# FunAudioLLM/CosyVoice

Measured on NVIDIA H100. Metric: audio-sec/s, CosyVoice2-0.5B zero-shot batch-32, NFE=10, higher is better.
Workload: dtype bf16

## Files before the change

cosyvoice_b200/csrc/api.cu:

```cuda
#include "common.cuh"
#include <string.h>
#include <algorithm>

void hift_build(cvk_ctx* ctx);
void hift_f0(cvk_ctx* ctx, const float* mel, const int* lens, int B, float* f0_out, cudaStream_t st);
void hift_source(cvk_ctx* ctx, const float* f0, const int* lens, int B, const float* noise, float* source_out, cudaStream_t st);
void hift_decode(cvk_ctx* ctx, const float* mel, const int* lens, int B, const float* source, float* wav, cudaStream_t st);
void hift_inference(cvk_ctx* ctx, const float* mel, const int* lens, int B, const float* noise, const float* cache_source,
                    const int* cache_lens, float* wav, float* source_out, cudaStream_t st);
void flow_build(cvk_ctx* ctx, const int* cfg, int ncfg);
void flow_encoder(cvk_ctx* ctx, const int32_t* tokens, const int* lens, int B, int streaming, int context_len, float* h, cudaStream_t st);
void flow_estimator(cvk_ctx* ctx, const float* x, const float* mu, const float* t, const float* spks, const float* cond, const int* lens,
                    int B, int streaming, float* out, cudaStream_t st);
void flow_cfm_solve(cvk_ctx* ctx, const float* mu, const float* spks, const float* cond, const int* lens, int B, const float* z,
                    int n_timesteps, float cfg_rate, int streaming, float* out, cudaStream_t st);
void flow_inference(cvk_ctx* ctx, const int32_t* tokens, const int* token_lens, const float* prompt_feat, const int* prompt_feat_lens,
                    const float* embedding, int B, int n_timesteps, int streaming, int finalize, float* mel, cudaStream_t st);
void flow_set_noise(cvk_ctx* ctx, const float* noise_tm, int T, int on_device);
void llm_build(cvk_ctx* ctx, const int* cfg, int ncfg);
cvk_lm_session* llm_session_create(cvk_ctx* ctx, int max_batch, int max_context);
void llm_session_destroy(cvk_ctx* ctx, cvk_lm_session* s);
void hift3_build(cvk_ctx* ctx);
void hift3_set_noise(cvk_ctx* ctx, const float* rand_ini, const float* sine_noise, long long n, int on_device);
void hift3_inference(cvk_ctx* ctx, const float* mel, const int* lens, int B, int finalize, float* wav, float* f0_out, float* source_out,
// ... 36 lines not shown
  if (!ctx) return CVK_ERR_INVALID; \
  try {                          \
    cudaSetDevice(ctx->device);
#define CVK_API_END                                  \
    return CVK_OK;                                   \
  } catch (const CvkError& e) {                      \
    ctx->last_error = e.what();                      \
    return e.code;                                   \
  } catch (const std::exception& e) {                \
    ctx->last_error = std::string("internal: ") + e.what(); \
    return CVK_ERR_INVALID;                          \
  }

extern "C" {

const char* cvk_version(void) { return "libcvk 0.1 (sm_90a)"; }

int cvk_create(int device, int precision, size_t workspace_bytes, cvk_ctx** out) {
  if (!out) return CVK_ERR_INVALID;
  *out = nullptr;
  int n = 0;
  if (cudaGetDeviceCount(&n) != cudaSuccess || n <= device || device < 0) return CVK_ERR_CUDA;
  if (precision != CVK_PREC_FP32 && precision != CVK_PREC_BF16) return CVK_ERR_INVALID;
  if (cudaSetDevice(device) != cudaSuccess) return CVK_ERR_CUDA;
  cudaDeviceProp prop;
  if (cudaGetDeviceProperties(&prop, device) != cudaSuccess) return CVK_ERR_CUDA;
  if (prop.major != 9) return CVK_ERR_CUDA;
  cvk_ctx* ctx = new cvk_ctx();
  ctx->device = device;
  ctx->precision = precision;
  ctx->act_dtype = precision == CVK_PREC_BF16 ? DT_BF16 : DT_F32;
  ctx->num_sms = prop.multiProcessorCount;
  if (workspace_bytes == 0) workspace_bytes = (size_t)4 << 30;
  void* p = nullptr;
  if (cudaMalloc(&p, workspace_bytes) != cudaSuccess) {
    delete ctx;
    return CVK_ERR_OOM;
  }
  ctx->arena.base = (char*)p;
  ctx->arena.cap = workspace_bytes;
  *out = ctx;
  return CVK_OK;
}

void cvk_destroy(cvk_ctx* ctx) {
  if (!ctx) return;
  cudaSetDevice(ctx->device);
  cudaDeviceSynchronize();
  for (auto& kv : ctx->raw) cudaFree(kv.second.p);
  for (void* p : ctx->owned) cudaFree(p);
  cudaFree(ctx->arena.base);
  delete ctx;
}

const char* cvk_last_error(cvk_ctx* ctx) { return ctx ? ctx->last_error.c_str() : "null context"; }
thread_local int cvk_in_capture = 0;
int64_t cvk_launch_count(cvk_ctx* ctx) { return ctx ? ctx->launches.load() : 0; }
int cvk_stream_create(cvk_ctx* ctx, void** out) {
  CVK_API_BEGIN
  CVK_REQUIRE(out != nullptr, "cvk_stream_create: bad arguments");
  cudaStream_t s = nullptr;
  CVK_CHECK_CUDA(cudaStreamCreateWithFlags(&s, cudaStreamNonBlocking));
  *out = (void*)s;
  CVK_API_END
}
void cvk_stream_destroy(cvk_ctx* ctx, void* stream) {
  if (!ctx || !stream) return;
  cudaSetDevice(ctx->device);
  cudaStreamDestroy((cudaStream_t)stream);
}
double cvk_last_op_ms(cvk_ctx* ctx) { return ctx ? ctx->op_ms : 0.0; }
int cvk_debug_read(cvk_ctx* ctx, long long* out, int n) {
  if (!ctx || !ctx->tl || !out || n != 4096) return CVK_ERR_INVALID;
  cudaSetDevice(ctx->device);
  if (cudaMemcpy(out, ctx->tl, 4096 * sizeof(long long), cudaMemcpyDeviceToHost) != cudaSuccess) return CVK_ERR_CUDA;
  return CVK_OK;
}

int cvk_set_option(cvk_ctx* ctx, const char* key, int value) {
  CVK_API_BEGIN
  std::string k(key ? key : "");
  if (k == "use_tc") ctx->use_tc = value;
  else if (k == "flow_fused_ff") ctx->flow_fused_ff = value;
  else if (k == "tc_epi") ctx->tc_epi = value;
  else if (k == "tc_persist") ctx->tc_persist = value;
  else if (k == "op_out_bf16") ctx->op_out_bf16 = value;
  else if (k == "op_iters") ctx->op_iters = value;
  else if (k == "use_graph") ctx->use_graph = value;
  else if (k == "use_tc_attn") ctx->use_tc_attn = value;
  else if (k == "use_skinny") ctx->use_skinny = value;
  else if (k == "lm_fused") ctx->lm_fused = value;
  else if (k == "pdl") ctx->pdl = value;
  else if (k == "lm_mega") ctx->lm_mega = value;
  else if (k == "enc_tc_attn") ctx->enc_tc_attn = value;
  else if (k == "hift_f16") ctx->hift_f16 = value;
  else if (k == "mega_coop") ctx->mega_coop = value;
  else if (k == "chain_timeline") {
    if (value && !ctx->tl) {
      ctx->tl = ctx->dmalloc(4096 * sizeof(long long));
      CVK_CHECK_CUDA(cudaMemset(ctx->tl, 0, 4096 * sizeof(long long)));
    }
    if (!value) ctx->tl = nullptr;
  }
  else throw CvkError(CVK_ERR_INVALID, "unknown option: " + k);
  CVK_API_END
}

int cvk_profile(cvk_ctx* ctx, int enable) {
  CVK_API_BEGIN
  CVK_CHECK_CUDA(cudaDeviceSynchronize());
  for (auto& r : ctx->prof) { ctx->event_pool.push_back(r.a); ctx->event_pool.push_back(r.b); }
  ctx->prof.clear();
  ctx->prof_on = enable;
  CVK_API_END
}

int cvk_profile_read(cvk_ctx* ctx, int family, double* ms, double* flops, double* bytes, int64_t* launches) {
  CVK_API_BEGIN
  CVK_REQUIRE(family >= 0 && family < FAM_COUNT && ms && flops && bytes && launches, "cvk_profile_read: bad arguments");
  CVK_CHECK_CUDA(cudaDeviceSynchronize());
  double t = 0, w = 0, by = 0;
  int64_t n = 0;
  for (auto& r : ctx->prof) {
    if (r.family != family) continue;
    float e = 0.f;
    CVK_CHECK_CUDA(cudaEventElapsedTime(&e, r.a, r.b));
    t += e; w += r.work; by += r.bytes; ++n;
  }
  *ms = t; *flops = w; *bytes = by; *launches = n;
  CVK_API_END
}

int cvk_set_tensor(cvk_ctx* ctx, const char* name, const float* data, int on_device, const int64_t* shape, int ndim) {
  CVK_API_BEGIN
  CVK_REQUIRE(name && data && shape && ndim >= 1 && ndim <= 4, "cvk_set_tensor: bad arguments");
  RawTensor t;
  t.shape.assign(shape, shape + ndim);
  size_t bytes = (size_t)t.numel() * sizeof(float);
  CVK_CHECK_CUDA(cudaMalloc((void**)&t.p, bytes));
  cudaError_t e = cudaMemcpy(t.p, data, bytes, on_device ? cudaMemcpyDeviceToDevice : cudaMemcpyHostToDevice);
  if (e != cudaSuccess) {
    cudaFree(t.p);
    throw CvkError(CVK_ERR_CUDA, std::string("cvk_set_tensor copy: ") + cudaGetErrorString(e));
  }
  auto it = ctx->raw.find(name);
  if (it != ctx->raw.end()) {
    cudaFree(it->second.p);
    ctx->raw.erase(it);
  }
  ctx->raw[name] = t;
  CVK_API_END
}

int cvk_finalize(cvk_ctx* ctx, const char* stage, const int* cfg, int ncfg) {
  CVK_API_BEGIN
  std::string s(stage ? stage : "");
  if (s == "hift") hift_build(ctx);
  else if (s == "flow") flow_build(ctx, cfg, ncfg);
  else if (s == "flow3") dit_build(ctx, cfg, ncfg);
  else if (s == "hift3") hift3_build(ctx);
  else if (s == "llm") llm_build(ctx, cfg, ncfg);
  else if (s == "mel") mel_init(ctx);
  else if (s == "prompt") prompt_feat_init(ctx);
  else throw CvkError(CVK_ERR_INVALID, "unknown stage: " + s);
  CVK_CHECK_CUDA(cudaDeviceSynchronize());
  std::string prefix = s + ".";
// ... 632 lines not shown
```

cosyvoice_b200/csrc/cvk_internal.h:

```cpp
#pragma once
#include <cuda_runtime.h>
#include <cuda_bf16.h>
#include <cuda_fp16.h>
#include <cuda.h>
#include <stdint.h>
#include <stdio.h>
#include <string>
#include <vector>
#include <map>
#include <unordered_map>
#include <stdexcept>
#include <atomic>

#include "../../include/cvk.h"

typedef __nv_bfloat16 bf16;

struct CvkError : std::runtime_error {
  int code;
  CvkError(int c, const std::string& m) : std::runtime_error(m), code(c) {}
};

#define CVK_CHECK_CUDA(expr)                                                                       \
  do {                                                                                             \
// ... 73 lines not shown
extern thread_local int cvk_in_capture;

struct Arena {
  char* base = nullptr;
  size_t cap = 0, off = 0, high = 0;
  void* alloc(size_t bytes) {
    size_t a = (off + 255) & ~(size_t)255;
    if (a + bytes > cap) throw CvkError(CVK_ERR_OOM, "workspace arena exhausted: need " + std::to_string(a + bytes) +
                                                          " of " + std::to_string(cap));
    off = a + bytes;
    if (off > high) high = off;
    return base + a;
  }
  void reset() { off = 0; }
};

struct RawTensor {
  float* p = nullptr;
  std::vector<int64_t> shape;
  int64_t numel() const { int64_t n = 1; for (auto s : shape) n *= s; return n; }
};

enum ProfFamily { FAM_GEMM_TC = 0, FAM_GEMM_SIMT = 1, FAM_ATTN = 2, FAM_COUNT = 3 };
struct ProfRec {
  cudaEvent_t a, b;
  int family;
  double work;
  double bytes;
};

struct HiftModel;
struct FlowModel;
struct DitModel;
struct LlmModel;

struct cvk_ctx {
  int device = 0;
  int precision = CVK_PREC_FP32;
  int act_dtype = DT_F32;
  int num_sms = 132;
  std::string last_error;
  std::map<std::string, RawTensor> raw;
  std::vector<void*> owned;
  Arena arena;
  HiftModel* hift = nullptr;
  HiftModel* hift3 = nullptr;
  void* hift3_extra = nullptr;
  FlowModel* flow = nullptr;
  DitModel* dit = nullptr;
  LlmModel* llm = nullptr;
  void* mel_model = nullptr;
  void* prompt_feat_model = nullptr;
  void* encode_tiled = nullptr;
  std::atomic<int64_t> launches{0};
  int op_out_bf16 = 0;
  int op_iters = 0;
  double op_ms = 0.0;
  int tc_epi = 2;
  int tc_persist = 2;
  void* tl = nullptr;
  int tl_seq = 0;
  long long* tl_next() {
    if (!tl) return nullptr;
    long long* p = (long long*)tl + 4 * (tl_seq % 1024);
    ++tl_seq;
    return p;
  }
  int prof_on = 0;
  std::vector<ProfRec> prof;
  std::unordered_map<const void*, void*> tiled;
  std::vector<cudaEvent_t> event_pool;
  int pdl = 1;
  int lm_fused = 1;
  int hift_f16 = 1;
  int build_f16 = 0;
  int enc_tc_attn = 1;
  int lm_mega = 0;
  int mega_coop = 1;
  int use_skinny = 1;
  int use_tc_attn = 1;
  int use_graph = 1;
  int use_tc = 1;
  int flow_fused_ff = 1;

  void* dmalloc(size_t bytes) {
    void* p = nullptr;
    CVK_CHECK_CUDA(cudaMalloc(&p, bytes ? bytes : 16));
    owned.push_back(p);
    return p;
  }
  const RawTensor& get_raw(const std::string& name) const {
    auto it = raw.find(name);
    if (it == raw.end()) throw CvkError(CVK_ERR_MISSING_WEIGHT, "missing weight tensor: " + name);
    return it->second;
  }
  bool has_raw(const std::string& name) const { return raw.find(name) != raw.end(); }
};

template <typename... KArgs, typename... Args>
inline void launch_ex(void (*kern)(KArgs...), dim3 grid, dim3 block, size_t smem, cudaStream_t st, bool pdl, Args&&... args) {
  cudaLaunchConfig_t cfg = {};
  cfg.gridDim = grid;
  cfg.blockDim = block;
  cfg.dynamicSmemBytes = smem;
  cfg.stream = st;
  cudaLaunchAttribute at[1];
  if (pdl) {
    at[0].id = cudaLaunchAttributeProgrammaticStreamSerialization;
    at[0].val.programmaticStreamSerializationAllowed = 1;
    cfg.attrs = at;
    cfg.numAttrs = 1;
  }
  CVK_CHECK_CUDA(cudaLaunchKernelEx(&cfg, kern, KArgs(std::forward<Args>(args))...));
}

Seqs make_seqs(cvk_ctx* ctx, const int* lens, int B, int gap, int scale, int extra_front, cudaStream_t st, bool with_row2seq = true);
Seqs scale_seqs(cvk_ctx* ctx, const Seqs& s, int scale, int extra_front, cudaStream_t st, bool with_row2seq = true);

ConvW make_linear(cvk_ctx* ctx, const std::string& wname, const std::string& bname);
ConvW make_conv(cvk_ctx* ctx, const float* w_oik , const float* bias, int N, int K, int taps,
                int dil, int shift0);
ConvW make_conv_named(cvk_ctx* ctx, const std::string& wname, const std::string& bname, int dil, int shift0);
float* fold_weight_norm(cvk_ctx* ctx, const std::string& prefix, int64_t* numel_out);
void finish_convw(cvk_ctx* ctx, ConvW& w);
float* dev_copy_f32(cvk_ctx* ctx, const float* src_dev, size_t n);

void conv_gemm(cvk_ctx* ctx, cudaStream_t st, const Mat& A, const ConvW& W, const Epilogue& ep);
void conv_gemm_simt(cvk_ctx* ctx, cudaStream_t st, const Mat& A, const ConvW& W, const Epilogue& ep);
void conv_gemm_tc(cvk_ctx* ctx, cudaStream_t st, const Mat& A, const ConvW& W, const Epilogue& ep);
void ffn_fused(cvk_ctx* ctx, cudaStream_t st, const Mat& x, const int* row2seq, const float* ln3_g, const float* ln3_b, const ConvW& w1,
               const ConvW& w2, const float* ln_g, const float* ln_b, const Mat& out);
void flow_ff(cvk_ctx* ctx, cudaStream_t st, const Mat& x, const int* row2seq, const float* ln3_g, const float* ln3_b, const ConvW& ff1,
             const ConvW& ff2, const float* ln_g, const float* ln_b, const Mat& out, const Mat& xn, const Mat& hid);
size_t skinny_scratch_floats(int rows, int maxN);
const bf16* skinny_tiled_weights(cvk_ctx* ctx, const ConvW& W);
void skinny_set_carveout();
int conv_gemm_skinny_ex(cvk_ctx* ctx, cudaStream_t st, const Mat& A, const ConvW& W, const Epilogue& ep, float* scratch, size_t scratch_floats,
                        int mode);
void conv_gemm_skinny(cvk_ctx* ctx, cudaStream_t st, const Mat& A, const ConvW& W, const Epilogue& ep, float* scratch, size_t scratch_floats);

void zero_mat(cvk_ctx* ctx, cudaStream_t st, const Mat& m);
void layernorm(cvk_ctx* ctx, cudaStream_t st, const Mat& x, const float* gamma, const float* beta, float eps, int act,
               float post_scale, const int* row2seq, const Mat& out, const float* rowvec = nullptr, int rowvec_ld = 0);
void unpack_rows_skip(cvk_ctx* ctx, cudaStream_t st, const Mat& in, const Seqs& s, const int* skip_host, float* dense, int C);
Seqs shrink_seqs(cvk_ctx* ctx, const Seqs& s, int drop_tail, cudaStream_t st);
Seqs subseqs(cvk_ctx* ctx, const Seqs& s, const int* skip_host, cudaStream_t st);
void rmsnorm(cvk_ctx* ctx, cudaStream_t st, const Mat& x, const float* gamma, float eps, const Mat& out);
void act_copy(cvk_ctx* ctx, cudaStream_t st, const Mat& x, int act, float param, const float* alpha, const int* row2seq,
              const Mat& out);
void act_copy_scaled(cvk_ctx* ctx, cudaStream_t st, const Mat& x, float pre_scale, int act, float param, const float* alpha,
                     const int* row2seq, const Mat& out);
void pack_rows(cvk_ctx* ctx, cudaStream_t st, const float* dense, int C, const Seqs& s, const Mat& out);
void unpack_rows(cvk_ctx* ctx, cudaStream_t st, const Mat& in, const Seqs& s, int skip, float* dense, int C);
void bcast_rows(cvk_ctx* ctx, cudaStream_t st, const float* vec, int C, int vec_ld, const Seqs& s, const Mat& out);
void convert_mat(cvk_ctx* ctx, cudaStream_t st, const Mat& in, const Mat& out);

struct KvGeom {
  const int* d_kstart = nullptr;
  const int* d_klen = nullptr;
  const int* d_qoff = nullptr;
};
void whisper_log_mel(cvk_ctx* ctx, const float* wav, const int* lens, int B, float* out, cudaStream_t st);
void kaldi_fbank80(cvk_ctx* ctx, const float* wav, const int* lens, int B, int subtract_mean, float* out, cudaStream_t st);
struct cvk_flow_stream;
cvk_flow_stream* flow_stream_create(cvk_ctx* ctx, int kind, int slots, int max_frames, int n_timesteps);
void flow_stream_destroy(cvk_flow_stream* fs);
// ... 44 lines not shown
```

cosyvoice_b200/csrc/gemm_tc.cu:

```cuda
#include "common.cuh"
#include "wgmma.cuh"

namespace {

constexpr int TC_BM = 128;
constexpr int TC_BK = 64;
constexpr int TC_THREADS = 384;

__device__ __forceinline__ uint32_t smem_u32(const void* p) { return (uint32_t)__cvta_generic_to_shared(p); }

__device__ __forceinline__ void mbar_init(uint32_t bar, uint32_t count) {
  asm volatile("mbarrier.init.shared::cta.b64 [%0], %1;" ::"r"(bar), "r"(count));
}
__device__ __forceinline__ void mbar_expect_tx(uint32_t bar, uint32_t bytes) {
  asm volatile("mbarrier.arrive.expect_tx.shared::cta.b64 _, [%0], %1;" ::"r"(bar), "r"(bytes) : "memory");
}
__device__ __forceinline__ void mbar_wait(uint32_t bar, uint32_t parity) {
  uint32_t ok = 0;
  asm volatile(
      "{\n\t.reg .pred p;\n\t"
      "mbarrier.try_wait.parity.shared::cta.b64 p, [%1], %2;\n\t"
      "selp.u32 %0, 1, 0, p;\n\t}"
      : "=r"(ok)
      : "r"(bar), "r"(parity)
// ... 342 lines not shown
      wg_fence();
      if (ep.ab_f16) {
#pragma unroll
        for (int k = 0; k < TC_BK / 16; ++k) wgmma_ss<BN, 1>(acc, da + (uint64_t)(2 * k), db + (uint64_t)(2 * k), 1);
      } else {
#pragma unroll
        for (int k = 0; k < TC_BK / 16; ++k) wgmma_ss<BN, 0>(acc, da + (uint64_t)(2 * k), db + (uint64_t)(2 * k), 1);
      }
      wg_commit();
      wg_wait<1>();
      __syncwarp();
      if (i > 0 && lane == 0) mbar_arrive(smem_u32(&bar_empty[(it - 1) % NSTG]));
    }
    wg_wait<0>();
    wg_touch<BN / 2>(acc);
    __syncwarp();
    if (iters > 0 && lane == 0) mbar_arrive(smem_u32(&bar_empty[(it - 1) % NSTG]));
    asm volatile("bar.sync 1, 256;" ::: "memory");

    const uint32_t stg1 = stg_base;
    const uint32_t stg2 = stg_base + (uint32_t)TC_BM * BN * (ep.out_dtype == DT_F32 ? 4u : 2u);
#pragma unroll
    for (int cb = 0; cb < BN; cb += 32) {
      float a16[16], v[16], w2[16];
      wg_frag_rows16(acc + cb / 2, lane, a16);
      const int c = cb + cq;
      if (n0 + c < N) {
        if (epi_mode == 2) {
          if (n0 + c + 16 <= N) epi_math16p(ep, r, rin, seq, valid, s_bias, c, n0 + c, a16, v, w2);
          else epi_math16(ep, r, rin, n0 + c, N, a16, v, w2);
          stage_store16(stg1, ep.out_dtype, row, c, v);
          if (ep.out2) stage_store16(stg2, ep.out2_dtype, row, c, w2);
        } else if (rin) {
          epi_store16(ep, r, n0 + c, N, a16);
        }
      }
    }
    if (epi_mode == 2) {
      asm volatile("fence.proxy.async.shared::cta;" ::: "memory");
      asm volatile("bar.sync 1, 256;" ::: "memory");
      if (ct == 0) {
        const int w1 = ep.out_dtype == DT_F32 ? 32 : 64;
        for (int sb = 0; sb * w1 < BN && n0 + sb * w1 < N; ++sb) tma_store_2d(&tmap_o, stg1 + sb * 16384u, n0 + sb * w1, r0);
        if (ep.out2) {
          const int w2c = ep.out2_dtype == DT_F32 ? 32 : 64;
          for (int sb = 0; sb * w2c < BN && n0 + sb * w2c < N; ++sb) tma_store_2d(&tmap_o2, stg2 + sb * 16384u, n0 + sb * w2c, r0);
        }
        asm volatile("cp.async.bulk.commit_group;" ::: "memory");
      }
    }
  }
  if (ct == 0 && epi_mode == 2) asm volatile("cp.async.bulk.wait_group 0;" ::: "memory");
}

typedef CUresult (*EncodeTiledFn)(CUtensorMap*, CUtensorMapDataType, cuuint32_t, void*, const cuuint64_t*, const cuuint64_t*,
                                  const cuuint32_t*, const cuuint32_t*, CUtensorMapInterleave, CUtensorMapSwizzle,
                                  CUtensorMapL2promotion, CUtensorMapFloatOOBfill);

EncodeTiledFn get_encode(cvk_ctx* ctx) {
  if (!ctx->encode_tiled) {
    void* fn = nullptr;
    cudaDriverEntryPointQueryResult qres;
    CVK_CHECK_CUDA(cudaGetDriverEntryPoint("cuTensorMapEncodeTiled", &fn, cudaEnableDefault, &qres));
    CVK_REQUIRE(fn != nullptr && qres == cudaDriverEntryPointSuccess, "cuTensorMapEncodeTiled not available");
    ctx->encode_tiled = fn;
  }
  return (EncodeTiledFn)ctx->encode_tiled;
}

template <int BN, int NSTG>
void launch_wg(cvk_ctx* ctx, cudaStream_t st, const CUtensorMap& ta, const CUtensorMap& tw, const CUtensorMap& to, const CUtensorMap& to2,
               const ConvW& W, int rowsOut, const EpiDev& e, int epi_mode) {
  constexpr size_t smem = (size_t)NSTG * (TC_BM * TC_BK * 2 + BN * TC_BK * 2) + TC_STG_BYTES + 1024;
  static bool attr_set = false;
  if (!attr_set) {
    CVK_CHECK_CUDA(cudaFuncSetAttribute(conv_gemm_wg_kernel<BN, NSTG>, cudaFuncAttributeMaxDynamicSharedMemorySize, (int)smem));
    attr_set = true;
  }
  const int ntn = ceil_div(W.N, BN), ntiles = ntn * ceil_div(rowsOut, TC_BM);
  const int grid = (ctx->tc_persist && ntiles > ctx->num_sms) ? ctx->num_sms : ntiles;
  conv_gemm_wg_kernel<BN, NSTG><<<grid, TC_THREADS, smem, st>>>(ta, tw, to, to2, W.N, W.K, W.taps, W.dil, W.shift0, rowsOut, e, epi_mode, ntn, ntiles);
}

constexpr int FF_C = 256, FF_HID = 1024, FF_HC = 64, FF_NCH = FF_HID / FF_HC;
constexpr uint32_t FF_A_BYTES = TC_BM * FF_C * 2;
constexpr uint32_t FF_W1_BYTES = FF_HC * FF_C * 2;
constexpr uint32_t FF_W2_BYTES = FF_C * FF_HC * 2;
constexpr uint32_t FF_STAGE_BYTES = FF_W1_BYTES + FF_W2_BYTES;
constexpr int FF_NSTG = 2;
constexpr int FF_OLD = FF_C + 8;
constexpr size_t FF_SMEM = FF_A_BYTES + FF_NSTG * FF_STAGE_BYTES + 1024;
static_assert((size_t)TC_BM * FF_OLD * 4 <= FF_A_BYTES + FF_NSTG * FF_STAGE_BYTES, "output staging tile must fit the operand region");

struct FfnDev {
  float* x;
  int ldx, rows;
  const int* row2seq;
  const float *ln3_g, *ln3_b, *b1, *b2;
  const float *ln_g, *ln_b;
  bf16* out;
  int ldo;
};

__global__ void __launch_bounds__(TC_THREADS, 1)
ffn_fused_kernel(const __grid_constant__ CUtensorMap tmap_w1, const __grid_constant__ CUtensorMap tmap_w2, FfnDev p) {
  extern __shared__ uint8_t smem_raw[];
  __shared__ __align__(8) uint64_t bar_full[FF_NSTG];
  __shared__ __align__(8) uint64_t bar_empty[FF_NSTG];
  const uint32_t smem_base = (smem_u32(smem_raw) + 1023u) & ~1023u;
  const uint32_t w_base = smem_base + FF_A_BYTES;
  const int warp = threadIdx.x >> 5, lane = threadIdx.x & 31;
  const int r0 = blockIdx.x * TC_BM;

  if (threadIdx.x == 0) {
    for (int s = 0; s < FF_NSTG; ++s) {
      mbar_init(smem_u32(&bar_full[s]), 1);
      mbar_init(smem_u32(&bar_empty[s]), 8);
    }
    asm volatile("fence.mbarrier_init.release.cluster;" ::: "memory");
  }
  __syncthreads();

  if (warp < 4) {
    asm volatile("setmaxnreg.dec.sync.aligned.u32 40;" ::: "memory");
    if (warp == 0 && lane == 0) {
      for (int c = 0; c < FF_NCH; ++c) {
        const uint32_t s = c % FF_NSTG, round = c / FF_NSTG;
        mbar_wait(smem_u32(&bar_empty[s]), (round & 1u) ^ 1u);
        const uint32_t sw = w_base + s * FF_STAGE_BYTES;
        const uint32_t fb = smem_u32(&bar_full[s]);
        mbar_expect_tx(fb, FF_STAGE_BYTES);
#pragma unroll
        for (int kt = 0; kt < FF_C / 64; ++kt) tma_load_2d(sw + kt * (FF_HC * 128u), &tmap_w1, fb, kt * 64, c * FF_HC);
        tma_load_2d(sw + FF_W1_BYTES, &tmap_w2, fb, c * FF_HC, 0);
      }
    }
    return;
  }
  asm volatile("setmaxnreg.inc.sync.aligned.u32 232;" ::: "memory");
  const int ct = threadIdx.x - 128;
  const int wg = ct >> 7;
  const int cw = ct >> 5;
  const int c0 = lane * 4, c1 = 128 + lane * 4;

  for (int i = 0; i < 16; ++i) {
    const int row = cw * 16 + i, r = r0 + row;
    float v[8];
#pragma unroll
    for (int j = 0; j < 8; ++j) v[j] = 0.f;
    if (r < p.rows && p.row2seq[r] >= 0) {
      const float* xp = p.x + (size_t)r * p.ldx;
      const float4 a = *reinterpret_cast<const float4*>(xp + c0), b = *reinterpret_cast<const float4*>(xp + c1);
      v[0] = a.x; v[1] = a.y; v[2] = a.z; v[3] = a.w; v[4] = b.x; v[5] = b.y; v[6] = b.z; v[7] = b.w;
      ln256_warp(v, p.ln3_g, p.ln3_b, 1e-5f, c0, c1);
    }
#pragma unroll
    for (int h = 0; h < 2; ++h) {
      const int c = h ? c1 : c0;
      __nv_bfloat162 lo = __floats2bfloat162_rn(v[4 * h], v[4 * h + 1]), hi = __floats2bfloat162_rn(v[4 * h + 2], v[4 * h + 3]);
      const uint32_t addr = smem_base + (uint32_t)(c >> 6) * (TC_BM * 128u) + (uint32_t)row * 128u +
                            ((((uint32_t)(c & 63) >> 3) ^ (uint32_t)(row & 7)) << 4) + (uint32_t)(c & 7) * 2u;
      asm volatile("st.shared.v2.b32 [%0], {%1,%2};" ::"r"(addr), "r"(*reinterpret_cast<uint32_t*>(&lo)), "r"(*reinterpret_cast<uint32_t*>(&hi))
                   : "memory");
    }
  }
  asm volatile("fence.proxy.async.shared::cta;" ::: "memory");
// ... 52 lines not shown
    const int rb = wg * 64 + (warp & 3) * 16 + (lane >> 2);
#pragma unroll
    for (int j = 0; j < 32; ++j) {
      const int col = 8 * j + 2 * q;
      const float2 b = *reinterpret_cast<const float2*>(p.b2 + col);
      *reinterpret_cast<float2*>(stg + rb * FF_OLD + col) = make_float2(o[4 * j] + b.x, o[4 * j + 1] + b.y);
      *reinterpret_cast<float2*>(stg + (rb + 8) * FF_OLD + col) = make_float2(o[4 * j + 2] + b.x, o[4 * j + 3] + b.y);
    }
  }
  asm volatile("bar.sync 1, 256;" ::: "memory");

  for (int i = 0; i < 16; ++i) {
    const int row = cw * 16 + i, r = r0 + row;
    if (r >= p.rows) break;
    const bool valid = p.row2seq[r] >= 0;
    float* xp = p.x + (size_t)r * p.ldx;
    const float* sp = stg + row * FF_OLD;
    const float4 sa = *reinterpret_cast<const float4*>(sp + c0), sb = *reinterpret_cast<const float4*>(sp + c1);
    const float4 xa = *reinterpret_cast<const float4*>(xp + c0), xb = *reinterpret_cast<const float4*>(xp + c1);
    float v[8] = {sa.x + xa.x, sa.y + xa.y, sa.z + xa.z, sa.w + xa.w, sb.x + xb.x, sb.y + xb.y, sb.z + xb.z, sb.w + xb.w};
    if (!valid) {
#pragma unroll
      for (int j = 0; j < 8; ++j) v[j] = 0.f;
    }
    *reinterpret_cast<float4*>(xp + c0) = make_float4(v[0], v[1], v[2], v[3]);
    *reinterpret_cast<float4*>(xp + c1) = make_float4(v[4], v[5], v[6], v[7]);
    if (p.ln_g && valid) ln256_warp(v, p.ln_g, p.ln_b, 1e-5f, c0, c1);
    bf16* op = p.out + (size_t)r * p.ldo;
    __nv_bfloat162 h0 = __floats2bfloat162_rn(v[0], v[1]), h1 = __floats2bfloat162_rn(v[2], v[3]);
    __nv_bfloat162 h2 = __floats2bfloat162_rn(v[4], v[5]), h3 = __floats2bfloat162_rn(v[6], v[7]);
    *reinterpret_cast<uint2*>(op + c0) = make_uint2(*reinterpret_cast<uint32_t*>(&h0), *reinterpret_cast<uint32_t*>(&h1));
    *reinterpret_cast<uint2*>(op + c1) = make_uint2(*reinterpret_cast<uint32_t*>(&h2), *reinterpret_cast<uint32_t*>(&h3));
  }
}

}

void conv_gemm_tc(cvk_ctx* ctx, cudaStream_t st, const Mat& A, const ConvW& W, const Epilogue& ep) {
  CVK_REQUIRE((A.dtype == DT_BF16 && W.w16 != nullptr) || (A.dtype == DT_F16 && W.wf16 != nullptr), "conv_gemm_tc: 16-bit operands (A and W of the same kind) required");
  const void* w16p = A.dtype == DT_F16 ? (const void*)W.wf16 : (const void*)W.w16;
  CVK_REQUIRE(A.cols >= W.K, "conv_gemm_tc: A has fewer columns than K");
  CVK_REQUIRE(W.K % 8 == 0 && A.ld % 8 == 0 && ((uintptr_t)A.p & 15) == 0, "conv_gemm_tc: operands must be 16-byte aligned");
  CVK_REQUIRE(ep.out.p != nullptr && ep.out.cols >= W.N, "conv_gemm_tc: bad output");
  EncodeTiledFn enc = get_encode(ctx);
  const int BN = W.N > 64 ? 128 : 64;
  CUtensorMap ta, tw;
  {
    cuuint64_t dims[2] = {(cuuint64_t)W.K, (cuuint64_t)A.rows};
    cuuint64_t strides[1] = {(cuuint64_t)A.ld * 2};
    cuuint32_t box[2] = {TC_BK, TC_BM};
    cuuint32_t es[2] = {1, 1};
    CUresult r = enc(&ta, CU_TENSOR_MAP_DATA_TYPE_BFLOAT16, 2, A.p, dims, strides, box, es, CU_TENSOR_MAP_INTERLEAVE_NONE,
                     CU_TENSOR_MAP_SWIZZLE_128B, CU_TENSOR_MAP_L2_PROMOTION_L2_128B, CU_TENSOR_MAP_FLOAT_OOB_FILL_NONE);
    CVK_REQUIRE(r == CUDA_SUCCESS, "cuTensorMapEncodeTiled(A) failed: " + std::to_string((int)r));
  }
  {
    cuuint64_t dims[3] = {(cuuint64_t)W.K, (cuuint64_t)W.taps, (cuuint64_t)W.N};
    cuuint64_t strides[2] = {(cuuint64_t)W.K * 2, (cuuint64_t)W.K * W.taps * 2};
    cuuint32_t box[3] = {TC_BK, 1, (cuuint32_t)BN};
    cuuint32_t es[3] = {1, 1, 1};
    CUresult r = enc(&tw, CU_TENSOR_MAP_DATA_TYPE_BFLOAT16, 3, const_cast<void*>(w16p), dims, strides, box, es, CU_TENSOR_MAP_INTERLEAVE_NONE,
                     CU_TENSOR_MAP_SWIZZLE_128B, CU_TENSOR_MAP_L2_PROMOTION_L2_256B, CU_TENSOR_MAP_FLOAT_OOB_FILL_NONE);
    CVK_REQUIRE(r == CUDA_SUCCESS, "cuTensorMapEncodeTiled(W) failed: " + std::to_string((int)r));
  }
  EpiDev e = to_dev(ep);
  e.ab_f16 = A.dtype == DT_F16;
  if (!e.bias) e.bias = W.bias;
  int rowsOut = ep.out.rows;
  CVK_REQUIRE((ep.out.ld * ep.out.esize()) % 16 == 0 && ((uintptr_t)ep.out.p & 15) == 0, "conv_gemm_tc: output rows must be 16-byte aligned");
  CVK_REQUIRE(!ep.resid.p || (ep.resid.ld % 4 == 0 && ((uintptr_t)ep.resid.p & 15) == 0), "conv_gemm_tc: residual alignment");
  CVK_REQUIRE(!(ep.resid.p && ep.rowvec), "conv_gemm_tc: residual and per-sequence vector cannot be combined");
  CVK_REQUIRE(!ep.rowvec || (ep.rowvec_ld % 4 == 0 && ((uintptr_t)ep.rowvec & 15) == 0), "conv_gemm_tc: rowvec alignment");
  CVK_REQUIRE(!ep.out2.p || ((ep.out2.ld * ep.out2.esize()) % 16 == 0 && ((uintptr_t)ep.out2.p & 15) == 0), "conv_gemm_tc: out2 alignment");
  const double flops = 2.0 * rowsOut * (double)W.N * W.K * W.taps;
  const double bytes = (double)rowsOut * W.K * 2 + (double)W.N * W.K * W.taps * 2 + (double)rowsOut * W.N * ep.out.esize();
  ProfScope ps(ctx, st, FAM_GEMM_TC, flops, bytes);
  int epi_mode = ctx->tc_epi == 2 ? 2 : 0;
  CUtensorMap to = ta, to2 = ta;
  if (epi_mode == 2) {
    const size_t need = (size_t)TC_BM * BN * ep.out.esize() + (ep.out2.p ? (size_t)TC_BM * BN * ep.out2.esize() : 0);
    const bool whole16 = (W.N * ep.out.esize()) % 16 == 0 && (!ep.out2.p || (W.N * ep.out2.esize()) % 16 == 0);
    if (ep.accumulate || need > TC_STG_BYTES || !whole16) epi_mode = 0;
  }
  if (epi_mode == 2) {
    auto mk = [&](CUtensorMap* m, const Mat& o) {
      cuuint64_t dims[2] = {(cuuint64_t)W.N, (cuuint64_t)rowsOut};
      cuuint64_t strides[1] = {(cuuint64_t)o.ld * o.esize()};
      cuuint32_t box[2] = {(cuuint32_t)(o.dtype == DT_F32 ? 32 : 64), TC_BM};
      cuuint32_t es[2] = {1, 1};
      CUresult r = enc(m, o.dtype == DT_F32 ? CU_TENSOR_MAP_DATA_TYPE_FLOAT32 : CU_TENSOR_MAP_DATA_TYPE_BFLOAT16, 2, o.p, dims, strides, box, es,
                       CU_TENSOR_MAP_INTERLEAVE_NONE, CU_TENSOR_MAP_SWIZZLE_128B, CU_TENSOR_MAP_L2_PROMOTION_NONE, CU_TENSOR_MAP_FLOAT_OOB_FILL_NONE);
      CVK_REQUIRE(r == CUDA_SUCCESS, "cuTensorMapEncodeTiled(out) failed: " + std::to_string((int)r));
    };
    mk(&to, ep.out);
    if (ep.out2.p) mk(&to2, ep.out2);
  }
  if (BN == 128) launch_wg<128, 4>(ctx, st, ta, tw, to, to2, W, rowsOut, e, epi_mode);
  else launch_wg<64, 4>(ctx, st, ta, tw, to, to2, W, rowsOut, e, epi_mode);
  ctx->launches++;
  CVK_LAUNCH_CHECK();
}

void ffn_fused(cvk_ctx* ctx, cudaStream_t st, const Mat& x, const int* row2seq, const float* ln3_g, const float* ln3_b, const ConvW& w1,
               const ConvW& w2, const float* ln_g, const float* ln_b, const Mat& out) {
  CVK_REQUIRE(x.dtype == DT_F32 && x.cols == FF_C && x.ld % 4 == 0 && ((uintptr_t)x.p & 15) == 0, "ffn_fused: x must be fp32 [rows, 256], 16-byte aligned rows");
  CVK_REQUIRE(out.dtype == DT_BF16 && out.cols == FF_C && out.rows >= x.rows && out.ld % 8 == 0 && ((uintptr_t)out.p & 15) == 0,
              "ffn_fused: out must be bf16 [rows, 256], 16-byte aligned rows");
  CVK_REQUIRE(w1.N == FF_HID && w1.K == FF_C && w1.taps == 1 && w1.w16 && w1.bias && w2.N == FF_C && w2.K == FF_HID && w2.taps == 1 && w2.w16 &&
                  w2.bias && row2seq && ln3_g && ln3_b && (!ln_g || ln_b),
              "ffn_fused: unexpected weights");
  CVK_REQUIRE((((uintptr_t)ln3_g | (uintptr_t)ln3_b | (uintptr_t)ln_g | (uintptr_t)ln_b | (uintptr_t)w1.bias | (uintptr_t)w2.bias) & 15) == 0,
              "ffn_fused: LayerNorm and bias vectors must be 16-byte aligned");
  EncodeTiledFn enc = get_encode(ctx);
  CUtensorMap t1, t2;
  auto mk = [&](CUtensorMap* m, const bf16* w, int N, int K, int box_n) {
    cuuint64_t dims[2] = {(cuuint64_t)K, (cuuint64_t)N};
    cuuint64_t strides[1] = {(cuuint64_t)K * 2};
    cuuint32_t box[2] = {64, (cuuint32_t)box_n};
    cuuint32_t es[2] = {1, 1};
    CUresult r = enc(m, CU_TENSOR_MAP_DATA_TYPE_BFLOAT16, 2, const_cast<bf16*>(w), dims, strides, box, es, CU_TENSOR_MAP_INTERLEAVE_NONE,
                     CU_TENSOR_MAP_SWIZZLE_128B, CU_TENSOR_MAP_L2_PROMOTION_L2_256B, CU_TENSOR_MAP_FLOAT_OOB_FILL_NONE);
    CVK_REQUIRE(r == CUDA_SUCCESS, "cuTensorMapEncodeTiled(ffn weights) failed: " + std::to_string((int)r));
  };
  mk(&t1, w1.w16, FF_HID, FF_C, FF_HC);
  mk(&t2, w2.w16, FF_C, FF_HID, FF_C);
  FfnDev p;
  p.x = x.f32(); p.ldx = x.ld; p.rows = x.rows; p.row2seq = row2seq;
  p.ln3_g = ln3_g; p.ln3_b = ln3_b; p.b1 = w1.bias; p.b2 = w2.bias; p.ln_g = ln_g; p.ln_b = ln_b;
  p.out = out.b16(); p.ldo = out.ld;
  const double flops = 4.0 * x.rows * (double)FF_C * FF_HID;
  const double bytes = (double)x.rows * FF_C * (4 + 4 + 2) + 2.0 * FF_C * FF_HID * 2;
  ProfScope ps(ctx, st, FAM_GEMM_TC, flops, bytes);
  static bool attr_set = false;
  if (!attr_set) {
    CVK_CHECK_CUDA(cudaFuncSetAttribute(ffn_fused_kernel, cudaFuncAttributeMaxDynamicSharedMemorySize, (int)FF_SMEM));
    attr_set = true;
  }
  ffn_fused_kernel<<<ceil_div(x.rows, TC_BM), TC_THREADS, FF_SMEM, st>>>(t1, t2, p);
  ctx->launches++;
  CVK_LAUNCH_CHECK();
}
```

Before: 415.9.

## Add A-panel-resident QKV GEMM kernel with streamed weight chunks for K=256

Adds a specialized warp-specialized WGMMA kernel for K=256 projections (e.g. flow QKV). It loads each 128-row activation panel once into shared memory and streams 128-column weight chunks through a two-stage pipeline. Two accumulator sets overlap the MMA for one chunk with the epilogue and TMA store of the previous. The intent is to cut repeated activation loads and per-tile pipeline overhead compared with the generic tiled GEMM. It only runs when the shape and epilogue conditions hold and there are enough row panels. The cost is a large new kernel with a heuristic for grouping column chunks.

```diff
diff --git a/cosyvoice_b200/csrc/api.cu b/cosyvoice_b200/csrc/api.cu
--- a/cosyvoice_b200/csrc/api.cu
+++ b/cosyvoice_b200/csrc/api.cu
@@ -142,6 +142,7 @@
   std::string k(key ? key : "");
   if (k == "use_tc") ctx->use_tc = value;
   else if (k == "flow_fused_ff") ctx->flow_fused_ff = value;
+  else if (k == "flow_qkv_panel") ctx->flow_qkv_panel = value;
   else if (k == "tc_epi") ctx->tc_epi = value;
   else if (k == "tc_persist") ctx->tc_persist = value;
   else if (k == "op_out_bf16") ctx->op_out_bf16 = value;
diff --git a/cosyvoice_b200/csrc/cvk_internal.h b/cosyvoice_b200/csrc/cvk_internal.h
--- a/cosyvoice_b200/csrc/cvk_internal.h
+++ b/cosyvoice_b200/csrc/cvk_internal.h
@@ -179,6 +179,7 @@
   int use_graph = 1;
   int use_tc = 1;
   int flow_fused_ff = 1;
+  int flow_qkv_panel = 1;
 
   void* dmalloc(size_t bytes) {
     void* p = nullptr;
diff --git a/cosyvoice_b200/csrc/gemm_tc.cu b/cosyvoice_b200/csrc/gemm_tc.cu
--- a/cosyvoice_b200/csrc/gemm_tc.cu
+++ b/cosyvoice_b200/csrc/gemm_tc.cu
@@ -448,6 +448,186 @@
   conv_gemm_wg_kernel<BN, NSTG><<<grid, TC_THREADS, smem, st>>>(ta, tw, to, to2, W.N, W.K, W.taps, W.dil, W.shift0, rowsOut, e, epi_mode, ntn, ntiles);
 }
 
+constexpr int QP_K = 256, QP_BN = 128, QP_NSTG = 2;
+constexpr uint32_t QP_A_BYTES = TC_BM * QP_K * 2;
+constexpr uint32_t QP_W_BYTES = QP_BN * QP_K * 2;
+constexpr uint32_t QP_STG_BYTES = TC_BM * QP_BN * 2;
+constexpr size_t QP_SMEM = QP_A_BYTES + QP_NSTG * QP_W_BYTES + QP_STG_BYTES + 1024;
+constexpr int QP_MIN_PANELS = 25;
+
+__global__ void __launch_bounds__(TC_THREADS, 1)
+qkv_panel_kernel(const __grid_constant__ CUtensorMap tmap_a, const __grid_constant__ CUtensorMap tmap_w,
+                 const __grid_constant__ CUtensorMap tmap_o, int shift0, int rowsOut, EpiDev ep, int ngroups, int cpu, int nunits) {
+  extern __shared__ uint8_t smem_raw[];
+  __shared__ __align__(8) uint64_t bar_full[QP_NSTG];
+  __shared__ __align__(8) uint64_t bar_empty[QP_NSTG];
+  __shared__ __align__(8) uint64_t bar_a_full, bar_a_empty;
+  __shared__ __align__(16) float s_bias_all[2 * QP_BN];
+  const uint32_t smem_base = (smem_u32(smem_raw) + 1023u) & ~1023u;
+  const uint32_t w_base = smem_base + QP_A_BYTES;
+  const uint32_t stg_base = w_base + QP_NSTG * QP_W_BYTES;
+  const int warp = threadIdx.x >> 5, lane = threadIdx.x & 31;
+
+  if (threadIdx.x == 0) {
+    for (int s = 0; s < QP_NSTG; ++s) {
+      mbar_init(smem_u32(&bar_full[s]), 1);
+      mbar_init(smem_u32(&bar_empty[s]), 8);
+    }
+    mbar_init(smem_u32(&bar_a_full), 1);
+    mbar_init(smem_u32(&bar_a_empty), 8);
+    asm volatile("fence.mbarrier_init.release.cluster;" ::: "memory");
+  }
+  __syncthreads();
+
+  if (warp < 4) {
+    asm volatile("setmaxnreg.dec.sync.aligned.u32 40;" ::: "memory");
+    if (warp == 0 && lane == 0) {
+      uint32_t it = 0, ui = 0;
+      for (int u = blockIdx.x; u < nunits; u += gridDim.x, ++ui) {
+        const int r0 = (u / ngroups) * TC_BM, c0 = (u % ngroups) * cpu;
+        for (int c = 0; c < cpu; ++c, ++it) {
+          const uint32_t s = it % QP_NSTG, round = it / QP_NSTG;
+          mbar_wait(smem_u32(&bar_empty[s]), (round & 1u) ^ 1u);
+          const uint32_t sw = w_base + s * QP_W_BYTES;
+          const uint32_t fb = smem_u32(&bar_full[s]);
+          mbar_expect_tx(fb, QP_W_BYTES);
+#pragma unroll
+          for (int kt = 0; kt < QP_K / TC_BK; ++kt) tma_load_3d(sw + kt * (QP_BN * 128u), &tmap_w, fb, kt * TC_BK, 0, (c0 + c) * QP_BN);
+          if (c == 0) {
+            mbar_wait(smem_u32(&bar_a_empty), (ui & 1u) ^ 1u);
+            const uint32_t fa = smem_u32(&bar_a_full);
+            mbar_expect_tx(fa, QP_A_BYTES);
+#pragma unroll
+            for (int kt = 0; kt < QP_K / TC_BK; ++kt) tma_load_2d(smem_base + kt * (TC_BM * 128u), &tmap_a, fa, kt * TC_BK, r0 + shift0);
+          }
+        }
+      }
+    }
+    return;
+  }
+  asm volatile("setmaxnreg.inc.sync.aligned.u32 232;" ::: "memory");
+  const int ct = threadIdx.x - 128;
+  const int wg = ct >> 7;
+  const int wt = ct & 127;
+  const int q = lane & 3;
+  const int row = wg * 64 + (warp & 3) * 16 + (lane >> 2) + 8 * (q & 1);
+  const int cq = 16 * (q >> 1);
+  const uint32_t a_wg = smem_base + (uint32_t)wg * (64 * 128u);
+  float* s_bias = s_bias_all + wg * QP_BN;
+  EpiDev e = ep;
+  e.out2 = nullptr;
+
+  int r0 = 0, r = 0, seq = 0;
+  bool rin = false, valid = false;
+  auto issue = [&](float* acc, uint32_t it) {
+    const uint32_t s = it % QP_NSTG;
+    mbar_wait(smem_u32(&bar_full[s]), (it / QP_NSTG) & 1u);
+    const uint32_t sw = w_base + s * QP_W_BYTES;
+#pragma unroll
+    for (int i = 0; i < QP_BN / 2; ++i) acc[i] = 0.f;
+    wg_fence();
+#pragma unroll
+    for (int kt = 0; kt < QP_K / TC_BK; ++kt) {
+      const uint64_t da = wg_desc_sw128(a_wg + kt * (TC_BM * 128u)), db = wg_desc_sw128(sw + kt * (QP_BN * 128u));
+      if (e.ab_f16) {
+#pragma unroll
+        for (int k = 0; k < TC_BK / 16; ++k) wgmma_ss<QP_BN, 1>(acc, da + (uint64_t)(2 * k), db + (uint64_t)(2 * k), 1);
+      } else {
+#pragma unroll
+        for (int k = 0; k < TC_BK / 16; ++k) wgmma_ss<QP_BN, 0>(acc, da + (uint64_t)(2 * k), db + (uint64_t)(2 * k), 1);
+      }
+    }
+    wg_commit();
+  };
+  auto release = [&](uint32_t it, bool last) {
+    __syncwarp();
+    if (lane == 0) {
+      mbar_arrive(smem_u32(&bar_empty[it % QP_NSTG]));
+      if (last) mbar_arrive(smem_u32(&bar_a_empty));
+    }
+  };
+  auto epilogue = [&](float* acc, int n0, float bv) {
+    if (wt == 0) asm volatile("cp.async.bulk.wait_group.read 0;" ::: "memory");
+    s_bias[wt] = bv;
+    asm volatile("bar.sync %0, 128;" ::"r"(2 + wg) : "memory");
+#pragma unroll
+    for (int cb = 0; cb < QP_BN; cb += 32) {
+      float a16[16], v[16], w2[16];
+      wg_frag_rows16(acc + cb / 2, lane, a16);
+      const int c = cb + cq;
+      epi_math16p(e, r, rin, seq, valid, s_bias, c, n0 + c, a16, v, w2);
+      stage_store16(stg_base, e.out_dtype, row, c, v);
+    }
+    asm volatile("fence.proxy.async.shared::cta;" ::: "memory");
+    asm volatile("bar.sync %0, 128;" ::"r"(2 + wg) : "memory");
+    if (wt == 0) {
+#pragma unroll
+      for (int sb = 0; sb < QP_BN / 64; ++sb)
+        tma_store_2d(&tmap_o, stg_base + sb * 16384u + (uint32_t)wg * 8192u, n0 + sb * 64, r0 + wg * 64);
+      asm volatile("cp.async.bulk.commit_group;" ::: "memory");
+    }
+  };
+
+  float acc0[QP_BN / 2], acc1[QP_BN / 2];
+  uint32_t it = 0, ui = 0;
+  for (int u = blockIdx.x; u < nunits; u += gridDim.x, ++ui) {
+    r0 = (u / ngroups) * TC_BM;
+    const int nb = (u % ngroups) * cpu * QP_BN;
+    r = r0 + row;
+    rin = r < rowsOut;
+    seq = 0;
+    if (rin && e.row2seq) seq = e.row2seq[r];
+    valid = rin && (!e.row2seq || seq >= 0);
+    mbar_wait(smem_u32(&bar_a_full), ui & 1u);
+    issue(acc0, it);
+    for (int c = 0; c < cpu; c += 2) {
+      float bv = e.bias ? e.bias[nb + c * QP_BN + wt] : 0.f;
+      if (c + 1 < cpu) {
+        issue(acc1, it + 1);
+        wg_wait<1>();
+      } else {
+        wg_wait<0>();
+      }
+      wg_touch<QP_BN / 2>(acc0);
+      release(it, c + 1 == cpu);
+      epilogue(acc0, nb + c * QP_BN, bv);
+      ++it;
+      if (c + 1 == cpu) break;
+      bv = e.bias ? e.bias[nb + (c + 1) * QP_BN + wt] : 0.f;
+      if (c + 2 < cpu) {
+        issue(acc0, it + 1);
+        wg_wait<1>();
+      } else {
+        wg_wait<0>();
+      }
+      wg_touch<QP_BN / 2>(acc1);
+      release(it, c + 2 == cpu);
+      epilogue(acc1, nb + (c + 1) * QP_BN, bv);
+      ++it;
+    }
+  }
+  if (wt == 0) asm volatile("cp.async.bulk.wait_group 0;" ::: "memory");
+}
+
+void launch_panel(cvk_ctx* ctx, cudaStream_t st, const CUtensorMap& ta, const CUtensorMap& tw, const CUtensorMap& to, const ConvW& W, int rowsOut,
+                  const EpiDev& e) {
+  static bool attr_set = false;
+  if (!attr_set) {
+    CVK_CHECK_CUDA(cudaFuncSetAttribute(qkv_panel_kernel, cudaFuncAttributeMaxDynamicSharedMemorySize, (int)QP_SMEM));
+    attr_set = true;
+  }
+  const int panels = ceil_div(rowsOut, TC_BM), nch = W.N / QP_BN;
+  int ngroups = 1;
+  long best = -1;
+  for (int g = 1; g <= 4; ++g) {
+    if (nch % g) continue;
+    const long cost = (long)ceil_div(panels * g, ctx->num_sms) * (nch / g + 1);
+    if (best < 0 || cost < best) { best = cost; ngroups = g; }
+  }
+  const int nunits = panels * ngroups;
+  qkv_panel_kernel<<<std::min(nunits, ctx->num_sms), TC_THREADS, QP_SMEM, st>>>(ta, tw, to, W.shift0, rowsOut, e, ngroups, nch / ngroups, nunits);
+}
+
 constexpr int FF_C = 256, FF_HID = 1024, FF_HC = 64, FF_NCH = FF_HID / FF_HC;
 constexpr uint32_t FF_A_BYTES = TC_BM * FF_C * 2;
 constexpr uint32_t FF_W1_BYTES = FF_HC * FF_C * 2;
@@ -666,11 +846,13 @@
     const bool whole16 = (W.N * ep.out.esize()) % 16 == 0 && (!ep.out2.p || (W.N * ep.out2.esize()) % 16 == 0);
     if (ep.accumulate || need > TC_STG_BYTES || !whole16) epi_mode = 0;
   }
+  const bool panel = ctx->flow_qkv_panel && epi_mode == 2 && W.taps == 1 && W.K == QP_K && W.N % QP_BN == 0 && W.N >= 512 && !ep.out2.p &&
+                     ep.out.esize() == 2 && (ctx->flow_qkv_panel == 2 || ceil_div(rowsOut, TC_BM) >= QP_MIN_PANELS);
   if (epi_mode == 2) {
     auto mk = [&](CUtensorMap* m, const Mat& o) {
       cuuint64_t dims[2] = {(cuuint64_t)W.N, (cuuint64_t)rowsOut};
       cuuint64_t strides[1] = {(cuuint64_t)o.ld * o.esize()};
-      cuuint32_t box[2] = {(cuuint32_t)(o.dtype == DT_F32 ? 32 : 64), TC_BM};
+      cuuint32_t box[2] = {(cuuint32_t)(o.dtype == DT_F32 ? 32 : 64), (cuuint32_t)(panel ? TC_BM / 2 : TC_BM)};
       cuuint32_t es[2] = {1, 1};
       CUresult r = enc(m, o.dtype == DT_F32 ? CU_TENSOR_MAP_DATA_TYPE_FLOAT32 : CU_TENSOR_MAP_DATA_TYPE_BFLOAT16, 2, o.p, dims, strides, box, es,
                        CU_TENSOR_MAP_INTERLEAVE_NONE, CU_TENSOR_MAP_SWIZZLE_128B, CU_TENSOR_MAP_L2_PROMOTION_NONE, CU_TENSOR_MAP_FLOAT_OOB_FILL_NONE);
@@ -679,7 +861,8 @@
     mk(&to, ep.out);
     if (ep.out2.p) mk(&to2, ep.out2);
   }
-  if (BN == 128) launch_wg<128, 4>(ctx, st, ta, tw, to, to2, W, rowsOut, e, epi_mode);
+  if (panel) launch_panel(ctx, st, ta, tw, to, W, rowsOut, e);
+  else if (BN == 128) launch_wg<128, 4>(ctx, st, ta, tw, to, to2, W, rowsOut, e, epi_mode);
   else launch_wg<64, 4>(ctx, st, ta, tw, to, to2, W, rowsOut, e, epi_mode);
   ctx->launches++;
   CVK_LAUNCH_CHECK();
```

Result: faster. 430.0 (median of 6 runs) (+3.4%).
